# jonasBoss/ndarray-interp

Measured on NVIDIA B200. Metric: queries/s, higher is better.
Workload: dtype f64

## Files before the change

ndarray_interp_b200/csrc/ndi_device.cuh:

```cuda
#pragma once

#include <cuda_runtime.h>
#include <stdint.h>

#include <type_traits>

#include "ndi_internal.h"

namespace ndi {

template <class T> struct Ar;
template <> struct Ar<float> {
    static __device__ __forceinline__ float add(float a, float b) { return __fadd_rn(a, b); }
    static __device__ __forceinline__ float sub(float a, float b) { return __fsub_rn(a, b); }
    static __device__ __forceinline__ float mul(float a, float b) { return __fmul_rn(a, b); }
    static __device__ __forceinline__ float div(float a, float b) { return __fdiv_rn(a, b); }
    static __device__ __forceinline__ float fma(float a, float b, float c) { return __fmaf_rn(a, b, c); }
    static __device__ __forceinline__ bool is_nan(float a) { return a != a; }
    static __device__ __forceinline__ bool is_finite(float a) { return isfinite(a); }
};
template <> struct Ar<double> {
    static __device__ __forceinline__ double add(double a, double b) { return __dadd_rn(a, b); }
    static __device__ __forceinline__ double sub(double a, double b) { return __dsub_rn(a, b); }
    static __device__ __forceinline__ double mul(double a, double b) { return __dmul_rn(a, b); }
// ... 142 lines not shown
struct Slope {
    T d;
    static __device__ __forceinline__ Slope make(T d, T , bool ) { return Slope{d}; }
    __device__ __forceinline__ Slope from_lane(int src) const { return Slope{__shfl_sync(0xffffffffu, d, src)}; }
    __device__ __forceinline__ Slope from_lane(int src, T, bool) const { return from_lane(src); }
};
template <>
struct Slope<float> {
    float d, r;
    static __device__ __forceinline__ Slope make(float d, float dq, bool tables_ok) {
        const bool ok = tables_ok && d >= 0x1p-40f && d <= 0x1p40f && fabsf(dq) <= 0x1p20f * d;
        return Slope{d, ok ? rcp_refined(d) : 0.0f};
    }
    __device__ __forceinline__ Slope from_lane(int src) const {
        return Slope{__shfl_sync(0xffffffffu, d, src), __shfl_sync(0xffffffffu, r, src)};
    }
    __device__ __forceinline__ Slope from_lane(int src, float dq_s, bool tables_ok) const {
#if NDI_PACK_SHFL >= 2
        return make(__shfl_sync(0xffffffffu, d, src), dq_s, tables_ok);
#else
        return from_lane(src);
#endif
    }
};

template <>
struct Slope<double> {
    double d, r;
    static __device__ __forceinline__ Slope make(double d, double , bool enabled) {
        const bool ok = enabled && d >= 0x1p-500 && d <= 0x1p500;
        return Slope{d, ok ? rcp_refined(d) : 0.0};
    }
    __device__ __forceinline__ Slope from_lane(int src) const {
        return Slope{__shfl_sync(0xffffffffu, d, src), __shfl_sync(0xffffffffu, r, src)};
    }
    __device__ __forceinline__ Slope from_lane(int src, double dq_s, bool enabled) const {
#if NDI_PACK_SHFL >= 2
        return make(__shfl_sync(0xffffffffu, d, src), dq_s, enabled);
#else
        return from_lane(src);
#endif
    }
    __device__ __forceinline__ double div(double a) const {
        const double q = div_by(a, d, r);
        return div_ok(a, q) ? q : __ddiv_rn(a, d);
    }
};

template <class T, int V> struct alignas(sizeof(T) * V) Vec { T v[V]; };

template <class T, int V>
__device__ __forceinline__ Vec<T, V> ld_table(const T* p) {
    Vec<T, V> r;
    if constexpr (sizeof(T) * V == 16) {
        int4 t = __ldg(reinterpret_cast<const int4*>(p));
        r = *reinterpret_cast<Vec<T, V>*>(&t);
    } else if constexpr (sizeof(T) * V == 8) {
        int2 t = __ldg(reinterpret_cast<const int2*>(p));
        r = *reinterpret_cast<Vec<T, V>*>(&t);
    } else {
        static_assert(sizeof(T) * V == 4, "unsupported vector width");
        int t = __ldg(reinterpret_cast<const int*>(p));
        r = *reinterpret_cast<Vec<T, V>*>(&t);
    }
    return r;
}
#ifndef NDI_STORE_MODE
#define NDI_STORE_MODE 0
#endif
template <class T, int V>
__device__ __forceinline__ void st_stream(T* p, const Vec<T, V>& r) {
#if NDI_STORE_MODE == 1
    if constexpr (sizeof(T) * V == 16) { *reinterpret_cast<int4*>(p) = *reinterpret_cast<const int4*>(&r); return; }
#elif NDI_STORE_MODE == 2
    if constexpr (sizeof(T) * V == 16) { __stwt(reinterpret_cast<int4*>(p), *reinterpret_cast<const int4*>(&r)); return; }
#elif NDI_STORE_MODE == 3
    if constexpr (sizeof(T) * V == 16) { __stcg(reinterpret_cast<int4*>(p), *reinterpret_cast<const int4*>(&r)); return; }
#endif
    if constexpr (sizeof(T) * V == 16) __stcs(reinterpret_cast<int4*>(p), *reinterpret_cast<const int4*>(&r));
    else if constexpr (sizeof(T) * V == 8) __stcs(reinterpret_cast<int2*>(p), *reinterpret_cast<const int2*>(&r));
    else __stcs(reinterpret_cast<int*>(p), *reinterpret_cast<const int*>(&r));
}
template <class T>
__device__ __forceinline__ T ld_query(const T* p) { return __ldcs(p); }

template <class T, int V>
__device__ __forceinline__ Vec<T, V> lerp_vec(const Vec<T, V>& y1, const Vec<T, V>& y2, const Slope<T>& s, T dq) {
    Vec<T, V> res;
    if constexpr (std::is_same<T, float>::value) {
        if (s.r != 0.0f) {
            if constexpr (NDI_F32X2 && V % 2 == 0) {
                const F2 r2 = F2::both(s.r), nb2 = F2::both(-s.d), dq2 = F2::both(dq);
#pragma unroll
                for (int e = 0; e < V; e += 2) {
                    const F2 a{y1.v[e], y1.v[e + 1]}, b{y2.v[e], y2.v[e + 1]};
                    const F2 o = add_halves(mul2(div_by2(sub2(b, a), nb2, r2), dq2), a);
                    res.v[e] = o.lo; res.v[e + 1] = o.hi;
                }
                return res;
            }
#pragma unroll
            for (int e = 0; e < V; ++e) {
                const float m = div_by(__fsub_rn(y2.v[e], y1.v[e]), s.d, s.r);
                res.v[e] = __fadd_rn(__fmul_rn(m, dq), y1.v[e]);
            }
            return res;
        }
    }
    if constexpr (std::is_same<T, double>::value) {
        if (s.r != 0.0) {
#pragma unroll
            for (int e = 0; e < V; ++e) res.v[e] = __dadd_rn(__dmul_rn(s.div(__dsub_rn(y2.v[e], y1.v[e])), dq), y1.v[e]);
            return res;
        }
    }
#pragma unroll
    for (int e = 0; e < V; ++e) res.v[e] = calc_frac_pre<T>(y1.v[e], y2.v[e], s.d, dq);
    return res;
}

template <class T, int V, bool PACK = true>
__device__ __forceinline__ Vec<T, V> bilerp_vec(const Vec<T, V>& z11, const Vec<T, V>& z12, const Vec<T, V>& z21,
                                                const Vec<T, V>& z22, const Slope<T>& sx, T dqx, const Slope<T>& sy, T dqy) {
    Vec<T, V> res;
    if constexpr (std::is_same<T, float>::value) {
        if (sx.r != 0.0f && sy.r != 0.0f) {
            bool all_ok = true;
            if constexpr (NDI_F32X2 && PACK && V % 2 == 0) {
                const F2 rx = F2::both(sx.r), nbx = F2::both(-sx.d), ry = F2::both(sy.r), nby = F2::both(-sy.d);
                const F2 dx2 = F2::both(dqx), dy2 = F2::both(dqy);
#pragma unroll
                for (int e = 0; e < V; e += 2) {
// ... 298 lines not shown
```

ndarray_interp_b200/csrc/ndi_eval.cu:

```cuda
#include <initializer_list>

#include "ndi_device.cuh"
#include "ndi_internal.h"

namespace ndi {

constexpr int kBlock = 256;
constexpr int kWarpsPerBlock = kBlock / 32;

template <class T>
struct Eval1 {
    const T* grid; int n; SearchCfg sc;
    const T* data; const T* a; const T* b; long long w;
    const T* q; long long nq; int mode;
    T* out; unsigned long long* err;
    long long ntasks; int nslices;
    int fast_tables;
};
template <class T>
struct Eval2 {
    const T* gx; int n; SearchCfg scx;
    const T* gy; int m; SearchCfg scy;
    const T* data; long long w;
    const T* qx; const T* qy; long long nq; int extrapolate;
// ... 252 lines not shown
    const long long want = (total + 255) / 256, cap = (long long)device_info().sm_count * 16;
    pack_pairs_kernel<T><<<(unsigned)(want < cap ? (want ? want : 1) : cap), 256, 0, st>>>(y, (long long)n, (long long)w, P);
    count_launch();
    return cudaGetLastError();
}
bool pair_table_shape_ok(int64_t w, size_t elem) {
    const int64_t v = 16 / (int64_t)elem;
    const int64_t lanes = w / v;
    return w % v == 0 && (lanes == 1 || lanes == 2 || lanes == 4);
}

template <class T>
__device__ __forceinline__ T rem_euclid(T a, T b) {
    T r = fmod(a, b);
    return r < (T)0 ? Ar<T>::add(r, fabs(b)) : r;
}

template <class T>
__device__ __forceinline__ T cubic_point(T yl, T yr, T al, T bl, T t, T omt, T tt) {
    const T lin = Ar<T>::add(Ar<T>::mul(omt, yl), Ar<T>::mul(t, yr));
    const T cur = Ar<T>::add(Ar<T>::mul(al, omt), Ar<T>::mul(bl, t));
    return Ar<T>::add(lin, Ar<T>::mul(tt, cur));
}

template <class T, int V>
__device__ __forceinline__ Vec<T, V> cubic_vec(const Vec<T, V>& yl, const Vec<T, V>& yr, const Vec<T, V>& al, const Vec<T, V>& bl,
                                               T t, T omt, T tt) {
    Vec<T, V> res;
    if constexpr (std::is_same<T, float>::value && NDI_F32X2 && V % 2 == 0) {
        const F2 t2 = F2::both(t), o2 = F2::both(omt), tt2 = F2::both(tt);
#pragma unroll
        for (int e = 0; e < V; e += 2) {
            const F2 l{yl.v[e], yl.v[e + 1]}, r{yr.v[e], yr.v[e + 1]}, a{al.v[e], al.v[e + 1]}, b{bl.v[e], bl.v[e + 1]};
            const F2 lin = add_halves(mul2(o2, l), mul2(t2, r));
            const F2 cur = add_halves(mul2(a, o2), mul2(b, t2));
            const F2 o = add_halves(lin, mul2(tt2, cur));
            res.v[e] = o.lo; res.v[e + 1] = o.hi;
        }
        return res;
    }
#pragma unroll
    for (int e = 0; e < V; ++e) res.v[e] = cubic_point<T>(yl.v[e], yr.v[e], al.v[e], bl.v[e], t, omt, tt);
    return res;
}

template <class T>
__device__ __forceinline__ bool cubic_prepare(T& x, T g0, T gl, int mode) {
    const bool inr = in_range(g0, gl, x);
    if (mode == 0) return !inr;
    if (mode == 2 && !inr) x = Ar<T>::add(rem_euclid<T>(Ar<T>::sub(x, g0), Ar<T>::sub(gl, g0)), g0);
    return Ar<T>::is_nan(x);
}

template <class T, int V, int LPQ>
__global__ void __launch_bounds__(kBlock, (sizeof(T) == 4 && LPQ < 32) ? NDI_THIN_MINBLOCKS : 0) interp1d_cubic_kernel(const Eval1<T> p) {
    extern __shared__ __align__(16) unsigned char smem_raw[];
    __shared__ uint64_t bar;
    const GridView<T> g = make_grid_view<T>(p.grid, p.n, p.sc, smem_raw, &bar);
    const T g0 = g.g0, gl = g.gl;
    const T one = (T)1;
    const int lane = threadIdx.x & 31;
    const long long nwarps = (long long)gridDim.x * kWarpsPerBlock;
    const long long task0 = (long long)blockIdx.x * kWarpsPerBlock + (threadIdx.x >> 5);
    T x_ahead = g0;
    if (LPQ < 32 && kTilesCubic == 1 && task0 < p.ntasks && task0 * 32 + lane < p.nq) x_ahead = ld_query(p.q + task0 * 32 + lane);
    for (long long task = task0; task < p.ntasks; task += nwarps) {
        if constexpr (LPQ < 32) {
            constexpr int TPW = kTilesCubic, QPR = 32 / LPQ;
            const long long qbase0 = task * (32 * TPW);
            T x[TPW]; int idx[TPW]; T tq[TPW], omt[TPW], tt[TPW]; bool skip[TPW], bad[TPW];
            if constexpr (TPW == 1) {
                x[0] = x_ahead;
                const long long qn = (task + nwarps) * 32 + lane;
                x_ahead = (task + nwarps < p.ntasks && qn < p.nq) ? ld_query(p.q + qn) : g0;
                bad[0] = cubic_prepare<T>(x[0], g0, gl, p.mode) && qbase0 + lane < p.nq;
            } else {
#pragma unroll
                for (int t = 0; t < TPW; ++t) {
                    const long long qi = qbase0 + t * 32 + lane;
                    const bool live = qi < p.nq;
                    x[t] = live ? ld_query(p.q + qi) : g0;
                    bad[t] = cubic_prepare<T>(x[t], g0, gl, p.mode) && live;
                }
            }
            search_multi<T, TPW>(g, x, idx, tq, omt);
#pragma unroll
            for (int t = 0; t < TPW; ++t) {
                const long long qi = qbase0 + t * 32 + lane;
                const T xl = tq[t], xr = omt[t];
                tq[t] = Ar<T>::div(Ar<T>::sub(x[t], xl), Ar<T>::sub(xr, xl));
                omt[t] = Ar<T>::sub(one, tq[t]);
                tt[t] = Ar<T>::mul(tq[t], omt[t]);
                if (qbase0 + t * 32 < p.nq) report_first_bad(p.err, bad[t], (unsigned long long)qi);
                skip[t] = bad[t] || !(qi < p.nq);
            }
            const int sub = lane % LPQ, qsel = lane / LPQ;
            const long long col = (long long)sub * V;
            const bool colok = col < p.w;
#pragma unroll
            for (int t = 0; t < TPW; ++t) {
                const long long qbase = qbase0 + t * 32;
                if (qbase >= p.nq) break;
                const int idx0 = __shfl_sync(0xffffffffu, idx[t], __ffs(__ballot_sync(0xffffffffu, !skip[t]) | 0x80000000u) - 1);
                const bool one_interval = LPQ > 1 && __all_sync(0xffffffffu, skip[t] || idx[t] == idx0);
                Vec<T, V> yl, yr, al, bl;
                if (one_interval && colok) {
                    const long long ro = (long long)idx0 * p.w + col;
                    yl = ld_table<T, V>(p.data + ro);
                    yr = ld_table<T, V>(p.data + ro + p.w);
                    al = ld_table<T, V>(p.a + ro);
                    bl = ld_table<T, V>(p.b + ro);
                }
#pragma unroll
                for (int r = 0; r < LPQ; ++r) {
                    const int src = r * QPR + qsel;
#if NDI_PACK_SHFL >= 1
                    const int is = __shfl_sync(0xffffffffu, skip[t] ? -1 : idx[t], src);
                    const bool live_s = is >= 0;
#else
                    const int is = __shfl_sync(0xffffffffu, idx[t], src);
                    const bool live_s = !shfl_b(skip[t], src);
#endif
#if NDI_PACK_CUBIC >= 2
                    const T ts = shfl_t(tq[t], src);
                    const T os = Ar<T>::sub(one, ts), tts = Ar<T>::mul(ts, os);
#else
                    const T ts = shfl_t(tq[t], src), os = shfl_t(omt[t], src), tts = shfl_t(tt[t], src);
#endif
                    if (live_s && colok) {
                        if (!one_interval) {
                            const long long ro = (long long)is * p.w + col;
                            yl = ld_table<T, V>(p.data + ro);
                            yr = ld_table<T, V>(p.data + ro + p.w);
                            al = ld_table<T, V>(p.a + ro);
                            bl = ld_table<T, V>(p.b + ro);
                        }
                        st_stream<T, V>(p.out + (qbase + src) * p.w + col, cubic_vec<T, V>(yl, yr, al, bl, ts, os, tts));
                    }
                }
            }
        } else {
            const long long tile = task / p.nslices;
            const int slice = (int)(task - tile * p.nslices);
            const long long qbase = tile * 32;
            const long long qi = qbase + lane;
            const bool live = qi < p.nq;
            T x[1] = {live ? ld_query(p.q + qi) : g0};
            const bool bad = cubic_prepare<T>(x[0], g0, gl, p.mode) && live;
            int idx[1]; T xls[1], xrs[1];
            search_multi<T, 1>(g, x, idx, xls, xrs);
            const T xl = xls[0], xr = xrs[0];
            const T t = Ar<T>::div(Ar<T>::sub(x[0], xl), Ar<T>::sub(xr, xl));
            const T omt = Ar<T>::sub(one, t);
            const T tt = Ar<T>::mul(t, omt);
            if (slice == 0) report_first_bad(p.err, bad, (unsigned long long)qi);
            const bool skip = bad || !live;
            const long long col = ((long long)slice * 32 + lane) * V;
            const bool colok = col < p.w;
            int cur = -1;
            Vec<T, V> yl, yr, al, bl;
            const int nlive = (int)min((long long)32, p.nq - qbase);
            for (int s = 0; s < nlive; ++s) {
                const int is = __shfl_sync(0xffffffffu, idx[0], s);
                const T ts = shfl_t(t, s), os = shfl_t(omt, s), tts = shfl_t(tt, s);
                const bool sk = shfl_b(skip, s);
                if (sk || !colok) continue;
                if (is != cur) {
                    const long long ro = (long long)is * p.w + col;
                    yl = ld_table<T, V>(p.data + ro);
                    yr = ld_table<T, V>(p.data + ro + p.w);
                    al = ld_table<T, V>(p.a + ro);
                    bl = ld_table<T, V>(p.b + ro);
                    cur = is;
                }
                st_stream<T, V>(p.out + (qbase + s) * p.w + col, cubic_vec<T, V>(yl, yr, al, bl, ts, os, tts));
            }
        }
    }
}

__device__ __forceinline__ F2 sub_halves(F2 p, F2 z) { return F2{__fsub_rn(p.lo, z.lo), __fsub_rn(p.hi, z.hi)}; }

template <class T, int ORDER>
__device__ __forceinline__ T cubic_deriv_point(T num, T h, T r) {
    if constexpr (ORDER == 1) return Hoisted<T>::div(num, h, r);
    else return Hoisted<T>::div(Hoisted<T>::div(num, h, r), h, r);
}

template <class T, int V, int ORDER>
__device__ __forceinline__ Vec<T, V> cubic_deriv_vec(const Vec<T, V>& yl, const Vec<T, V>& yr, const Vec<T, V>& al,
                                                     const Vec<T, V>& bl, T t, T omt, T h, T r) {
    const T dmt = Ar<T>::sub(omt, t), tt = Ar<T>::mul(t, omt);
    const T two = (T)2;
    Vec<T, V> res;
    if constexpr (std::is_same<T, float>::value && NDI_F32X2 && V % 2 == 0) {
        const F2 t2 = F2::both(t), o2 = F2::both(omt), d2 = F2::both(dmt), tt2 = F2::both(tt), two2 = F2::both(two);
#pragma unroll
        for (int e = 0; e < V; e += 2) {
            const F2 l{yl.v[e], yl.v[e + 1]}, rr{yr.v[e], yr.v[e + 1]}, a{al.v[e], al.v[e + 1]}, b{bl.v[e], bl.v[e + 1]};
            const F2 cur = add_halves(mul2(a, o2), mul2(b, t2));
            const F2 ba = sub2(b, a);
            F2 num;
            if constexpr (ORDER == 1) num = add_halves(mul2(tt2, ba), add_halves(mul2(d2, cur), sub2(rr, l)));
            else num = mul2(two2, sub_halves(mul2(d2, ba), cur));
            res.v[e] = cubic_deriv_point<T, ORDER>(num.lo, h, r);
            res.v[e + 1] = cubic_deriv_point<T, ORDER>(num.hi, h, r);
        }
        return res;
    }
#pragma unroll
    for (int e = 0; e < V; ++e) {
        const T cur = Ar<T>::add(Ar<T>::mul(al.v[e], omt), Ar<T>::mul(bl.v[e], t));
        const T ba = Ar<T>::sub(bl.v[e], al.v[e]);
        T num;
        if constexpr (ORDER == 1)
            num = Ar<T>::add(Ar<T>::add(Ar<T>::sub(yr.v[e], yl.v[e]), Ar<T>::mul(dmt, cur)), Ar<T>::mul(tt, ba));
        else num = Ar<T>::mul(two, Ar<T>::sub(Ar<T>::mul(dmt, ba), cur));
        res.v[e] = cubic_deriv_point<T, ORDER>(num, h, r);
    }
    return res;
}

template <class T, int V, int LPQ, int ORDER>
__global__ void __launch_bounds__(kBlock) interp1d_cubic_deriv_kernel(const Eval1<T> p) {
    extern __shared__ __align__(16) unsigned char smem_raw[];
    __shared__ uint64_t bar;
    const GridView<T> g = make_grid_view<T>(p.grid, p.n, p.sc, smem_raw, &bar);
    const T g0 = g.g0, gl = g.gl;
    const T one = (T)1;
// ... 407 lines not shown
            const T y = ld_query(qy + i);
            bady = (check == CHECK_IN_RANGE) ? !in_range(gy0, gyl, y) : Ar<T>::is_nan(y);
        }
        if (badx || bady) {
            unsigned long long word = qy ? 2ull * (unsigned long long)i + (badx ? 0ull : 1ull) : (unsigned long long)i;
            first = min(first, word);
        }
    }
#pragma unroll
    for (int o = 16; o > 0; o >>= 1) first = min(first, __shfl_xor_sync(0xffffffffu, first, o));
    if ((threadIdx.x & 31) == 0 && first != ~0ull) atomicMin(err, first);
}

static int pow2ceil(long long v) { int p = 1; while (p < v && p < 32) p <<= 1; return p; }

static bool aligned(const void* p, size_t a) { return ((uintptr_t)p % a) == 0; }

template <class T>
static int pick_vec(long long w, std::initializer_list<const void*> ptrs) {
    constexpr int vmax = 16 / (int)sizeof(T);
    for (int v = vmax; v > 1; v >>= 1) {
        bool ok = (w % v) == 0;
        for (const void* p : ptrs) ok = ok && aligned(p, sizeof(T) * v);
        if (ok) return v;
    }
    return 1;
}

struct Shape { int v; int lpq; int nslices; long long ntasks; };

static Shape pick_shape(long long w, long long nq, int v, int tiles_per_warp) {
    Shape s;
    s.v = v;
    long long groups = (w + v - 1) / v;
    s.lpq = pow2ceil(groups);
    long long tiles = (nq + 31) / 32;
    if (s.lpq == 32) {
        s.nslices = (int)((groups + 31) / 32);
        s.ntasks = tiles * s.nslices;
    } else {
        s.nslices = 1;
        s.ntasks = (tiles + tiles_per_warp - 1) / tiles_per_warp;
    }
    return s;
}

template <class K>
static cudaError_t prep_smem(K kernel, size_t bytes) {
    if (bytes > 30 * 1024) return cudaFuncSetAttribute(kernel, cudaFuncAttributeMaxDynamicSharedMemorySize, (int)bytes);
    return cudaSuccess;
}

template <class K>
static int persistent_grid(K kernel, size_t smem, long long ntasks) {
    int per_sm = 0;
    if (cudaOccupancyMaxActiveBlocksPerMultiprocessor(&per_sm, kernel, kBlock, smem) != cudaSuccess || per_sm < 1) per_sm = 1;
    long long want = (ntasks + kWarpsPerBlock - 1) / kWarpsPerBlock;
    long long cap = (long long)device_info().sm_count * per_sm;
    return (int)(want < cap ? (want < 1 ? 1 : want) : cap);
}

template <class P, class K>
static cudaError_t launch_eval(K kernel, const P& p, size_t smem, cudaStream_t st) {
    cudaError_t e = prep_smem(kernel, smem);
    if (e != cudaSuccess) return e;
    int grid = persistent_grid(kernel, smem, p.ntasks);
    kernel<<<grid, kBlock, smem, st>>>(p);
    count_launch();
    return cudaGetLastError();
}

#define NDI_LPQ_SWITCH(KERNEL, T, V, LPQ, P, SMEM, ST)                                   \
    switch (LPQ) {                                                                        \
    case 1:  return launch_eval(KERNEL<T, V, 1>, P, SMEM, ST);                            \
    case 2:  return launch_eval(KERNEL<T, V, 2>, P, SMEM, ST);                            \
    case 4:  return launch_eval(KERNEL<T, V, 4>, P, SMEM, ST);                            \
    case 8:  return launch_eval(KERNEL<T, V, 8>, P, SMEM, ST);                            \
    case 16: return launch_eval(KERNEL<T, V, 16>, P, SMEM, ST);                           \
    default: return launch_eval(KERNEL<T, V, 32>, P, SMEM, ST);                           \
    }

#define NDI_VEC_SWITCH(KERNEL, T, SH, P, SMEM, ST)                                        \
    if constexpr (sizeof(T) == 4) {                                                       \
        if (SH.v == 4) { NDI_LPQ_SWITCH(KERNEL, T, 4, SH.lpq, P, SMEM, ST) }              \
        if (SH.v == 2) { NDI_LPQ_SWITCH(KERNEL, T, 2, SH.lpq, P, SMEM, ST) }              \
        NDI_LPQ_SWITCH(KERNEL, T, 1, SH.lpq, P, SMEM, ST)                                 \
    } else {                                                                              \
        if (SH.v == 2) { NDI_LPQ_SWITCH(KERNEL, T, 2, SH.lpq, P, SMEM, ST) }              \
        NDI_LPQ_SWITCH(KERNEL, T, 1, SH.lpq, P, SMEM, ST)                                 \
    }

template <class T, int V, int LPQ> constexpr auto bilinear_direct = interp2d_bilinear_kernel<T, V, LPQ, false>;
template <class T, int V, int LPQ> constexpr auto bilinear_binned = interp2d_bilinear_kernel<T, V, LPQ, true>;

template <class T>
cudaError_t launch_interp1d_linear(const T* grid, int64_t n, SearchCfg sc, const T* data, int64_t w, const T* q,
                                   int64_t nq, int extrapolate, T* out, unsigned long long* err, int fast_tables,
                                   const T* pair, cudaStream_t st) {
    if (nq <= 0) return cudaSuccess;
    if (pair && pair_table_shape_ok(w, sizeof(T)) && aligned(out, 16)) {
        const long long tiles = (nq + 31) / 32;
        Eval1<T> p{grid, (int)n, sc, pair, nullptr, nullptr, (long long)w, q, (long long)nq, extrapolate, out, err, tiles, 1, fast_tables};
        const size_t smem = stage_bytes(sc, sizeof(T));
        switch ((int)(w / (16 / (int64_t)sizeof(T)))) {
        case 1: return launch_eval(interp1d_linear_pair_kernel<T, 1>, p, smem, st);
        case 2: return launch_eval(interp1d_linear_pair_kernel<T, 2>, p, smem, st);
        default: return launch_eval(interp1d_linear_pair_kernel<T, 4>, p, smem, st);
        }
    }
    Shape sh = pick_shape(w, nq, pick_vec<T>(w, {data, out}), kTilesLinear);
    Eval1<T> p{grid, (int)n, sc, data, nullptr, nullptr, (long long)w, q, (long long)nq, extrapolate, out, err, sh.ntasks, sh.nslices, fast_tables};
    size_t smem = stage_bytes(sc, sizeof(T));
    NDI_VEC_SWITCH(interp1d_linear_kernel, T, sh, p, smem, st)
}

template <class T>
cudaError_t launch_interp1d_cubic(const T* grid, int64_t n, SearchCfg sc, const T* data, const T* a, const T* b,
                                  int64_t w, const T* q, int64_t nq, int extrap_mode, T* out,
                                  unsigned long long* err, cudaStream_t st) {
    if (nq <= 0) return cudaSuccess;
    Shape sh = pick_shape(w, nq, pick_vec<T>(w, {data, a, b, out}), kTilesCubic);
    Eval1<T> p{grid, (int)n, sc, data, a, b, (long long)w, q, (long long)nq, extrap_mode, out, err, sh.ntasks, sh.nslices, 0};
    size_t smem = stage_bytes(sc, sizeof(T));
    NDI_VEC_SWITCH(interp1d_cubic_kernel, T, sh, p, smem, st)
}

template <class T, int V, int LPQ> constexpr auto cubic_deriv1 = interp1d_cubic_deriv_kernel<T, V, LPQ, 1>;
template <class T, int V, int LPQ> constexpr auto cubic_deriv2 = interp1d_cubic_deriv_kernel<T, V, LPQ, 2>;

template <class T>
cudaError_t launch_interp1d_cubic_deriv(const T* grid, int64_t n, SearchCfg sc, const T* data, const T* a, const T* b,
                                        int64_t w, const T* q, int64_t nq, int extrap_mode, int order, T* out,
                                        unsigned long long* err, cudaStream_t st) {
    if (nq <= 0) return cudaSuccess;
    Shape sh = pick_shape(w, nq, pick_vec<T>(w, {data, a, b, out}), 1);
    Eval1<T> p{grid, (int)n, sc, data, a, b, (long long)w, q, (long long)nq, extrap_mode, out, err, sh.ntasks, sh.nslices, 0};
    size_t smem = stage_bytes(sc, sizeof(T));
    if (order == 1) { NDI_VEC_SWITCH(cubic_deriv1, T, sh, p, smem, st) }
    NDI_VEC_SWITCH(cubic_deriv2, T, sh, p, smem, st)
}

template <class T>
cudaError_t launch_interp1d_linear_slope(const T* grid, int64_t n, SearchCfg sc, const T* data, int64_t w, const T* q,
                                         int64_t nq, int extrapolate, T* out, unsigned long long* err, cudaStream_t st) {
    if (nq <= 0) return cudaSuccess;
    Shape sh = pick_shape(w, nq, pick_vec<T>(w, {data, out}), 1);
    Eval1<T> p{grid, (int)n, sc, data, nullptr, nullptr, (long long)w, q, (long long)nq, extrapolate, out, err, sh.ntasks, sh.nslices, 0};
    size_t smem = stage_bytes(sc, sizeof(T));
    NDI_VEC_SWITCH(interp1d_linear_slope_kernel, T, sh, p, smem, st)
}

template <class T>
cudaError_t launch_interp2d_bilinear(const T* gx, int64_t n, SearchCfg scx, const T* gy, int64_t m, SearchCfg scy,
                                     const T* data, int64_t w, const T* qx, const T* qy, int64_t nq, int extrapolate,
                                     T* out, unsigned long long* err, const unsigned* perm, int fast_tables,
                                     unsigned long long* next_task, cudaStream_t st) {
    if (nq <= 0) return cudaSuccess;
    Shape sh = pick_shape(w, nq, pick_vec<T>(w, {data, out}), kTilesBilinear);
    Eval2<T> p{gx, (int)n, scx, gy, (int)m, scy, data, (long long)w, qx, qy, (long long)nq, extrapolate, out, err, sh.ntasks, sh.nslices, perm, fast_tables, perm ? next_task : nullptr};
    size_t smem = stage_bytes(scx, sizeof(T)) + stage_bytes(scy, sizeof(T));
    if (perm) { NDI_VEC_SWITCH(bilinear_binned, T, sh, p, smem, st) }
    NDI_VEC_SWITCH(bilinear_direct, T, sh, p, smem, st)
}

template <class T>
cudaError_t launch_lower_index(const T* grid, int64_t n, SearchCfg sc, const T* q, int64_t nq, int64_t* idx,
                               unsigned long long* err, cudaStream_t st) {
    if (nq <= 0) return cudaSuccess;
    size_t smem = stage_bytes(sc, sizeof(T));
    cudaError_t e = prep_smem(lower_index_kernel<T>, smem);
    if (e != cudaSuccess) return e;
    long long blocks = (nq + (long long)kBlock * 4 - 1) / ((long long)kBlock * 4);
    long long cap = (long long)device_info().sm_count * 8;
    lower_index_kernel<T><<<(int)(blocks < cap ? blocks : cap), kBlock, smem, st>>>(grid, (int)n, sc, q, (long long)nq,
                                                                                   (long long*)idx, err);
    count_launch();
    return cudaGetLastError();
// ... 49 lines not shown
```

Before: 707.8 million.

## Restructure wide-row cubic path into block-tiled two-phase kernel with 256-bit accesses

For wide rows (one query spread over a full warp), the cubic kernel now runs in two phases. First each thread of the block prepares one query (search, t, omt, tt) into shared memory. Then warps split the 256 queries and column slices between them, reusing loaded table rows when consecutive queries share an interval. It also adds 32-byte vector load/store paths (ld.global.nc.v4.u64 / st.global.cs.v4.u64) and changes the launch grid to one tile per block. The aim is to remove per-query shuffles and redundant searches across slices, at the cost of block-wide syncs and shared-memory traffic.

Result: slower. 688.5 million, median of 6 (-2.7%).

```diff
diff --git a/ndarray_interp_b200/csrc/ndi_device.cuh b/ndarray_interp_b200/csrc/ndi_device.cuh
--- a/ndarray_interp_b200/csrc/ndi_device.cuh
+++ b/ndarray_interp_b200/csrc/ndi_device.cuh
@@ -218,7 +218,11 @@
 template <class T, int V>
 __device__ __forceinline__ Vec<T, V> ld_table(const T* p) {
     Vec<T, V> r;
-    if constexpr (sizeof(T) * V == 16) {
+    if constexpr (sizeof(T) * V == 32) {
+        unsigned long long t[4];
+        asm("ld.global.nc.v4.u64 {%0,%1,%2,%3}, [%4];" : "=l"(t[0]), "=l"(t[1]), "=l"(t[2]), "=l"(t[3]) : "l"(p));
+        r = *reinterpret_cast<Vec<T, V>*>(t);
+    } else if constexpr (sizeof(T) * V == 16) {
         int4 t = __ldg(reinterpret_cast<const int4*>(p));
         r = *reinterpret_cast<Vec<T, V>*>(&t);
     } else if constexpr (sizeof(T) * V == 8) {
@@ -243,7 +247,10 @@
 #elif NDI_STORE_MODE == 3
     if constexpr (sizeof(T) * V == 16) { __stcg(reinterpret_cast<int4*>(p), *reinterpret_cast<const int4*>(&r)); return; }
 #endif
-    if constexpr (sizeof(T) * V == 16) __stcs(reinterpret_cast<int4*>(p), *reinterpret_cast<const int4*>(&r));
+    if constexpr (sizeof(T) * V == 32) {
+        const unsigned long long* u = reinterpret_cast<const unsigned long long*>(&r);
+        asm volatile("st.global.cs.v4.u64 [%0], {%1,%2,%3,%4};" ::"l"(p), "l"(u[0]), "l"(u[1]), "l"(u[2]), "l"(u[3]));
+    } else if constexpr (sizeof(T) * V == 16) __stcs(reinterpret_cast<int4*>(p), *reinterpret_cast<const int4*>(&r));
     else if constexpr (sizeof(T) * V == 8) __stcs(reinterpret_cast<int2*>(p), *reinterpret_cast<const int2*>(&r));
     else __stcs(reinterpret_cast<int*>(p), *reinterpret_cast<const int*>(&r));
 }
diff --git a/ndarray_interp_b200/csrc/ndi_eval.cu b/ndarray_interp_b200/csrc/ndi_eval.cu
--- a/ndarray_interp_b200/csrc/ndi_eval.cu
+++ b/ndarray_interp_b200/csrc/ndi_eval.cu
@@ -328,20 +328,79 @@
     return Ar<T>::is_nan(x);
 }
 
+constexpr int kCubicQB = kBlock;
+template <class T> struct alignas(16) CubicRec { T t, omt, tt; int is; };
+
+template <class T, int V>
+__device__ __forceinline__ void cubic_wide_rows(const Eval1<T>& p, const GridView<T>& g) {
+    static_assert(kCubicQB == kBlock, "phase 1 prepares one query per thread");
+    __shared__ CubicRec<T> recs[kCubicQB];
+    const T g0 = g.g0, gl = g.gl;
+    const T one = (T)1;
+    const int lane = threadIdx.x & 31, warp = threadIdx.x >> 5;
+    const int nsplit = max(1, kWarpsPerBlock / p.nslices);
+    const int units = p.nslices * nsplit;
+    for (long long tile = blockIdx.x; tile < p.ntasks; tile += gridDim.x) {
+        const long long qbase = tile * kCubicQB;
+        {
+            const long long qi = qbase + threadIdx.x;
+            const bool live = qi < p.nq;
+            T x[1] = {live ? ld_query(p.q + qi) : g0};
+            const bool bad = cubic_prepare<T>(x[0], g0, gl, p.mode) && live;
+            int idx[1]; T xls[1], xrs[1];
+            search_multi<T, 1>(g, x, idx, xls, xrs);
+            const T xl = xls[0], xr = xrs[0];
+            const T t = Ar<T>::div(Ar<T>::sub(x[0], xl), Ar<T>::sub(xr, xl));
+            const T omt = Ar<T>::sub(one, t);
+            const T tt = Ar<T>::mul(t, omt);
+            report_first_bad(p.err, bad, (unsigned long long)qi);
+            recs[threadIdx.x] = CubicRec<T>{t, omt, tt, (bad || !live) ? -1 : idx[0]};
+        }
+        __syncthreads();
+        const int nt = (int)min((long long)kCubicQB, p.nq - qbase);
+        for (int u = warp; u < units; u += kWarpsPerBlock) {
+            const int slice = u % p.nslices, part = u / p.nslices;
+            const long long col = ((long long)slice * 32 + lane) * V;
+            if (col >= p.w) continue;
+            const int s1 = (part + 1) * nt / nsplit;
+            int s = part * nt / nsplit;
+            T* o = p.out + (qbase + s) * p.w + col;
+            int cur = -1;
+            Vec<T, V> yl, yr, al, bl;
+            for (; s < s1; ++s, o += p.w) {
+                const CubicRec<T> r = recs[s];
+                if (r.is < 0) continue;
+                if (r.is != cur) {
+                    const long long ro = (long long)r.is * p.w + col;
+                    yl = ld_table<T, V>(p.data + ro);
+                    yr = ld_table<T, V>(p.data + ro + p.w);
+                    al = ld_table<T, V>(p.a + ro);
+                    bl = ld_table<T, V>(p.b + ro);
+                    cur = r.is;
+                }
+                st_stream<T, V>(o, cubic_vec<T, V>(yl, yr, al, bl, r.t, r.omt, r.tt));
+            }
+        }
+        __syncthreads();
+    }
+}
+
 template <class T, int V, int LPQ>
 __global__ void __launch_bounds__(kBlock, (sizeof(T) == 4 && LPQ < 32) ? NDI_THIN_MINBLOCKS : 0) interp1d_cubic_kernel(const Eval1<T> p) {
     extern __shared__ __align__(16) unsigned char smem_raw[];
     __shared__ uint64_t bar;
     const GridView<T> g = make_grid_view<T>(p.grid, p.n, p.sc, smem_raw, &bar);
-    const T g0 = g.g0, gl = g.gl;
-    const T one = (T)1;
-    const int lane = threadIdx.x & 31;
-    const long long nwarps = (long long)gridDim.x * kWarpsPerBlock;
-    const long long task0 = (long long)blockIdx.x * kWarpsPerBlock + (threadIdx.x >> 5);
-    T x_ahead = g0;
-    if (LPQ < 32 && kTilesCubic == 1 && task0 < p.ntasks && task0 * 32 + lane < p.nq) x_ahead = ld_query(p.q + task0 * 32 + lane);
-    for (long long task = task0; task < p.ntasks; task += nwarps) {
-        if constexpr (LPQ < 32) {
+    if constexpr (LPQ == 32) {
+        cubic_wide_rows<T, V>(p, g);
+    } else {
+        const T g0 = g.g0, gl = g.gl;
+        const T one = (T)1;
+        const int lane = threadIdx.x & 31;
+        const long long nwarps = (long long)gridDim.x * kWarpsPerBlock;
+        const long long task0 = (long long)blockIdx.x * kWarpsPerBlock + (threadIdx.x >> 5);
+        T x_ahead = g0;
+        if (kTilesCubic == 1 && task0 < p.ntasks && task0 * 32 + lane < p.nq) x_ahead = ld_query(p.q + task0 * 32 + lane);
+        for (long long task = task0; task < p.ntasks; task += nwarps) {
             constexpr int TPW = kTilesCubic, QPR = 32 / LPQ;
             const long long qbase0 = task * (32 * TPW);
             T x[TPW]; int idx[TPW]; T tq[TPW], omt[TPW], tt[TPW]; bool skip[TPW], bad[TPW];
@@ -414,42 +473,6 @@
                         st_stream<T, V>(p.out + (qbase + src) * p.w + col, cubic_vec<T, V>(yl, yr, al, bl, ts, os, tts));
                     }
                 }
-            }
-        } else {
-            const long long tile = task / p.nslices;
-            const int slice = (int)(task - tile * p.nslices);
-            const long long qbase = tile * 32;
-            const long long qi = qbase + lane;
-            const bool live = qi < p.nq;
-            T x[1] = {live ? ld_query(p.q + qi) : g0};
-            const bool bad = cubic_prepare<T>(x[0], g0, gl, p.mode) && live;
-            int idx[1]; T xls[1], xrs[1];
-            search_multi<T, 1>(g, x, idx, xls, xrs);
-            const T xl = xls[0], xr = xrs[0];
-            const T t = Ar<T>::div(Ar<T>::sub(x[0], xl), Ar<T>::sub(xr, xl));
-            const T omt = Ar<T>::sub(one, t);
-            const T tt = Ar<T>::mul(t, omt);
-            if (slice == 0) report_first_bad(p.err, bad, (unsigned long long)qi);
-            const bool skip = bad || !live;
-            const long long col = ((long long)slice * 32 + lane) * V;
-            const bool colok = col < p.w;
-            int cur = -1;
-            Vec<T, V> yl, yr, al, bl;
-            const int nlive = (int)min((long long)32, p.nq - qbase);
-            for (int s = 0; s < nlive; ++s) {
-                const int is = __shfl_sync(0xffffffffu, idx[0], s);
-                const T ts = shfl_t(t, s), os = shfl_t(omt, s), tts = shfl_t(tt, s);
-                const bool sk = shfl_b(skip, s);
-                if (sk || !colok) continue;
-                if (is != cur) {
-                    const long long ro = (long long)is * p.w + col;
-                    yl = ld_table<T, V>(p.data + ro);
-                    yr = ld_table<T, V>(p.data + ro + p.w);
-                    al = ld_table<T, V>(p.a + ro);
-                    bl = ld_table<T, V>(p.b + ro);
-                    cur = is;
-                }
-                st_stream<T, V>(p.out + (qbase + s) * p.w + col, cubic_vec<T, V>(yl, yr, al, bl, ts, os, tts));
             }
         }
     }
@@ -964,19 +987,19 @@
 }
 
 template <class K>
-static int persistent_grid(K kernel, size_t smem, long long ntasks) {
+static int persistent_grid(K kernel, size_t smem, long long ntasks, int tasks_per_block) {
     int per_sm = 0;
     if (cudaOccupancyMaxActiveBlocksPerMultiprocessor(&per_sm, kernel, kBlock, smem) != cudaSuccess || per_sm < 1) per_sm = 1;
-    long long want = (ntasks + kWarpsPerBlock - 1) / kWarpsPerBlock;
+    long long want = (ntasks + tasks_per_block - 1) / tasks_per_block;
     long long cap = (long long)device_info().sm_count * per_sm;
     return (int)(want < cap ? (want < 1 ? 1 : want) : cap);
 }
 
 template <class P, class K>
-static cudaError_t launch_eval(K kernel, const P& p, size_t smem, cudaStream_t st) {
+static cudaError_t launch_eval(K kernel, const P& p, size_t smem, cudaStream_t st, int tasks_per_block = kWarpsPerBlock) {
     cudaError_t e = prep_smem(kernel, smem);
     if (e != cudaSuccess) return e;
-    int grid = persistent_grid(kernel, smem, p.ntasks);
+    int grid = persistent_grid(kernel, smem, p.ntasks, tasks_per_block);
     kernel<<<grid, kBlock, smem, st>>>(p);
     count_launch();
     return cudaGetLastError();
@@ -1032,8 +1055,22 @@
                                   unsigned long long* err, cudaStream_t st) {
     if (nq <= 0) return cudaSuccess;
     Shape sh = pick_shape(w, nq, pick_vec<T>(w, {data, a, b, out}), kTilesCubic);
+    size_t smem = stage_bytes(sc, sizeof(T));
+    if (sh.lpq == 32) {
+        constexpr int v32 = 32 / (int)sizeof(T);
+        const bool wide32 = w % v32 == 0 && aligned(data, 32) && aligned(a, 32) && aligned(b, 32) && aligned(out, 32);
+        const int v = wide32 ? v32 : sh.v;
+        const long long slices = ((w + v - 1) / v + 31) / 32;
+        Eval1<T> p{grid, (int)n, sc, data, a, b, (long long)w, q, (long long)nq, extrap_mode, out, err,
+                   (nq + kCubicQB - 1) / kCubicQB, (int)slices, 0};
+        if (wide32) return launch_eval(interp1d_cubic_kernel<T, v32, 32>, p, smem, st, 1);
+        if constexpr (sizeof(T) == 4) {
+            if (v == 4) return launch_eval(interp1d_cubic_kernel<T, 4, 32>, p, smem, st, 1);
+        }
+        if (v == 2) return launch_eval(interp1d_cubic_kernel<T, 2, 32>, p, smem, st, 1);
+        return launch_eval(interp1d_cubic_kernel<T, 1, 32>, p, smem, st, 1);
+    }
     Eval1<T> p{grid, (int)n, sc, data, a, b, (long long)w, q, (long long)nq, extrap_mode, out, err, sh.ntasks, sh.nslices, 0};
-    size_t smem = stage_bytes(sc, sizeof(T));
     NDI_VEC_SWITCH(interp1d_cubic_kernel, T, sh, p, smem, st)
 }
 
```

## Split wide-row cubic into dedicated kernel with 256-bit loads/stores and smem records

Applied to the files above, without the earlier changes.

Moves the wide-row (LPQ==32) cubic path into its own kernel. That kernel stages per-query t/omt/tt/index records in shared memory instead of doing several warp shuffles per output row, processes two rows per iteration, and uses 32-byte vector global loads and streaming stores when alignment allows. The goal is fewer shuffles and fewer memory instructions per row of output. It relies on v4.f64/v8.f32 PTX (Blackwell-era) and adds shared-memory traffic plus a fixed minBlocks launch bound.

New measurement: 746.3 million before, 678.6 million after, median of 6. 9.1% lower.

```diff
diff --git a/ndarray_interp_b200/csrc/ndi_device.cuh b/ndarray_interp_b200/csrc/ndi_device.cuh
--- a/ndarray_interp_b200/csrc/ndi_device.cuh
+++ b/ndarray_interp_b200/csrc/ndi_device.cuh
@@ -218,7 +218,14 @@
 template <class T, int V>
 __device__ __forceinline__ Vec<T, V> ld_table(const T* p) {
     Vec<T, V> r;
-    if constexpr (sizeof(T) * V == 16) {
+    if constexpr (sizeof(T) * V == 32 && sizeof(T) == 8) {
+        asm("ld.global.nc.v4.f64 {%0, %1, %2, %3}, [%4];"
+            : "=d"(r.v[0]), "=d"(r.v[1]), "=d"(r.v[2]), "=d"(r.v[3]) : "l"(p));
+    } else if constexpr (sizeof(T) * V == 32) {
+        asm("ld.global.nc.v8.f32 {%0, %1, %2, %3, %4, %5, %6, %7}, [%8];"
+            : "=f"(r.v[0]), "=f"(r.v[1]), "=f"(r.v[2]), "=f"(r.v[3]), "=f"(r.v[4]), "=f"(r.v[5]), "=f"(r.v[6]), "=f"(r.v[7])
+            : "l"(p));
+    } else if constexpr (sizeof(T) * V == 16) {
         int4 t = __ldg(reinterpret_cast<const int4*>(p));
         r = *reinterpret_cast<Vec<T, V>*>(&t);
     } else if constexpr (sizeof(T) * V == 8) {
@@ -243,7 +250,14 @@
 #elif NDI_STORE_MODE == 3
     if constexpr (sizeof(T) * V == 16) { __stcg(reinterpret_cast<int4*>(p), *reinterpret_cast<const int4*>(&r)); return; }
 #endif
-    if constexpr (sizeof(T) * V == 16) __stcs(reinterpret_cast<int4*>(p), *reinterpret_cast<const int4*>(&r));
+    if constexpr (sizeof(T) * V == 32 && sizeof(T) == 8)
+        asm volatile("st.global.cs.v4.f64 [%0], {%1, %2, %3, %4};"
+                     :: "l"(p), "d"(r.v[0]), "d"(r.v[1]), "d"(r.v[2]), "d"(r.v[3]) : "memory");
+    else if constexpr (sizeof(T) * V == 32)
+        asm volatile("st.global.cs.v8.f32 [%0], {%1, %2, %3, %4, %5, %6, %7, %8};"
+                     :: "l"(p), "f"(r.v[0]), "f"(r.v[1]), "f"(r.v[2]), "f"(r.v[3]), "f"(r.v[4]), "f"(r.v[5]), "f"(r.v[6]),
+                        "f"(r.v[7]) : "memory");
+    else if constexpr (sizeof(T) * V == 16) __stcs(reinterpret_cast<int4*>(p), *reinterpret_cast<const int4*>(&r));
     else if constexpr (sizeof(T) * V == 8) __stcs(reinterpret_cast<int2*>(p), *reinterpret_cast<const int2*>(&r));
     else __stcs(reinterpret_cast<int*>(p), *reinterpret_cast<const int*>(&r));
 }
diff --git a/ndarray_interp_b200/csrc/ndi_eval.cu b/ndarray_interp_b200/csrc/ndi_eval.cu
--- a/ndarray_interp_b200/csrc/ndi_eval.cu
+++ b/ndarray_interp_b200/csrc/ndi_eval.cu
@@ -329,7 +329,8 @@
 }
 
 template <class T, int V, int LPQ>
-__global__ void __launch_bounds__(kBlock, (sizeof(T) == 4 && LPQ < 32) ? NDI_THIN_MINBLOCKS : 0) interp1d_cubic_kernel(const Eval1<T> p) {
+__global__ void __launch_bounds__(kBlock, sizeof(T) == 4 ? NDI_THIN_MINBLOCKS : 0) interp1d_cubic_kernel(const Eval1<T> p) {
+    static_assert(LPQ < 32, "wide rows: interp1d_cubic_wide_kernel");
     extern __shared__ __align__(16) unsigned char smem_raw[];
     __shared__ uint64_t bar;
     const GridView<T> g = make_grid_view<T>(p.grid, p.n, p.sc, smem_raw, &bar);
@@ -339,118 +340,150 @@
     const long long nwarps = (long long)gridDim.x * kWarpsPerBlock;
     const long long task0 = (long long)blockIdx.x * kWarpsPerBlock + (threadIdx.x >> 5);
     T x_ahead = g0;
-    if (LPQ < 32 && kTilesCubic == 1 && task0 < p.ntasks && task0 * 32 + lane < p.nq) x_ahead = ld_query(p.q + task0 * 32 + lane);
+    if (kTilesCubic == 1 && task0 < p.ntasks && task0 * 32 + lane < p.nq) x_ahead = ld_query(p.q + task0 * 32 + lane);
     for (long long task = task0; task < p.ntasks; task += nwarps) {
-        if constexpr (LPQ < 32) {
-            constexpr int TPW = kTilesCubic, QPR = 32 / LPQ;
-            const long long qbase0 = task * (32 * TPW);
-            T x[TPW]; int idx[TPW]; T tq[TPW], omt[TPW], tt[TPW]; bool skip[TPW], bad[TPW];
-            if constexpr (TPW == 1) {
-                x[0] = x_ahead;
-                const long long qn = (task + nwarps) * 32 + lane;
-                x_ahead = (task + nwarps < p.ntasks && qn < p.nq) ? ld_query(p.q + qn) : g0;
-                bad[0] = cubic_prepare<T>(x[0], g0, gl, p.mode) && qbase0 + lane < p.nq;
-            } else {
-#pragma unroll
-                for (int t = 0; t < TPW; ++t) {
-                    const long long qi = qbase0 + t * 32 + lane;
-                    const bool live = qi < p.nq;
-                    x[t] = live ? ld_query(p.q + qi) : g0;
-                    bad[t] = cubic_prepare<T>(x[t], g0, gl, p.mode) && live;
-                }
-            }
-            search_multi<T, TPW>(g, x, idx, tq, omt);
+        constexpr int TPW = kTilesCubic, QPR = 32 / LPQ;
+        const long long qbase0 = task * (32 * TPW);
+        T x[TPW]; int idx[TPW]; T tq[TPW], omt[TPW], tt[TPW]; bool skip[TPW], bad[TPW];
+        if constexpr (TPW == 1) {
+            x[0] = x_ahead;
+            const long long qn = (task + nwarps) * 32 + lane;
+            x_ahead = (task + nwarps < p.ntasks && qn < p.nq) ? ld_query(p.q + qn) : g0;
+            bad[0] = cubic_prepare<T>(x[0], g0, gl, p.mode) && qbase0 + lane < p.nq;
+        } else {
 #pragma unroll
             for (int t = 0; t < TPW; ++t) {
                 const long long qi = qbase0 + t * 32 + lane;
-                const T xl = tq[t], xr = omt[t];
-                tq[t] = Ar<T>::div(Ar<T>::sub(x[t], xl), Ar<T>::sub(xr, xl));
-                omt[t] = Ar<T>::sub(one, tq[t]);
-                tt[t] = Ar<T>::mul(tq[t], omt[t]);
-                if (qbase0 + t * 32 < p.nq) report_first_bad(p.err, bad[t], (unsigned long long)qi);
-                skip[t] = bad[t] || !(qi < p.nq);
-            }
-            const int sub = lane % LPQ, qsel = lane / LPQ;
-            const long long col = (long long)sub * V;
-            const bool colok = col < p.w;
-#pragma unroll
-            for (int t = 0; t < TPW; ++t) {
-                const long long qbase = qbase0 + t * 32;
-                if (qbase >= p.nq) break;
-                const int idx0 = __shfl_sync(0xffffffffu, idx[t], __ffs(__ballot_sync(0xffffffffu, !skip[t]) | 0x80000000u) - 1);
-                const bool one_interval = LPQ > 1 && __all_sync(0xffffffffu, skip[t] || idx[t] == idx0);
-                Vec<T, V> yl, yr, al, bl;
-                if (one_interval && colok) {
-                    const long long ro = (long long)idx0 * p.w + col;
-                    yl = ld_table<T, V>(p.data + ro);
-                    yr = ld_table<T, V>(p.data + ro + p.w);
-                    al = ld_table<T, V>(p.a + ro);
-                    bl = ld_table<T, V>(p.b + ro);
-                }
-#pragma unroll
-                for (int r = 0; r < LPQ; ++r) {
-                    const int src = r * QPR + qsel;
+                const bool live = qi < p.nq;
+                x[t] = live ? ld_query(p.q + qi) : g0;
+                bad[t] = cubic_prepare<T>(x[t], g0, gl, p.mode) && live;
+            }
+        }
+        search_multi<T, TPW>(g, x, idx, tq, omt);
+#pragma unroll
+        for (int t = 0; t < TPW; ++t) {
+            const long long qi = qbase0 + t * 32 + lane;
+            const T xl = tq[t], xr = omt[t];
+            tq[t] = Ar<T>::div(Ar<T>::sub(x[t], xl), Ar<T>::sub(xr, xl));
+            omt[t] = Ar<T>::sub(one, tq[t]);
+            tt[t] = Ar<T>::mul(tq[t], omt[t]);
+            if (qbase0 + t * 32 < p.nq) report_first_bad(p.err, bad[t], (unsigned long long)qi);
+            skip[t] = bad[t] || !(qi < p.nq);
+        }
+        const int sub = lane % LPQ, qsel = lane / LPQ;
+        const long long col = (long long)sub * V;
+        const bool colok = col < p.w;
+#pragma unroll
+        for (int t = 0; t < TPW; ++t) {
+            const long long qbase = qbase0 + t * 32;
+            if (qbase >= p.nq) break;
+            const int idx0 = __shfl_sync(0xffffffffu, idx[t], __ffs(__ballot_sync(0xffffffffu, !skip[t]) | 0x80000000u) - 1);
+            const bool one_interval = LPQ > 1 && __all_sync(0xffffffffu, skip[t] || idx[t] == idx0);
+            Vec<T, V> yl, yr, al, bl;
+            if (one_interval && colok) {
+                const long long ro = (long long)idx0 * p.w + col;
+                yl = ld_table<T, V>(p.data + ro);
+                yr = ld_table<T, V>(p.data + ro + p.w);
+                al = ld_table<T, V>(p.a + ro);
+                bl = ld_table<T, V>(p.b + ro);
+            }
+#pragma unroll
+            for (int r = 0; r < LPQ; ++r) {
+                const int src = r * QPR + qsel;
 #if NDI_PACK_SHFL >= 1
-                    const int is = __shfl_sync(0xffffffffu, skip[t] ? -1 : idx[t], src);
-                    const bool live_s = is >= 0;
+                const int is = __shfl_sync(0xffffffffu, skip[t] ? -1 : idx[t], src);
+                const bool live_s = is >= 0;
 #else
-                    const int is = __shfl_sync(0xffffffffu, idx[t], src);
-                    const bool live_s = !shfl_b(skip[t], src);
+                const int is = __shfl_sync(0xffffffffu, idx[t], src);
+                const bool live_s = !shfl_b(skip[t], src);
 #endif
 #if NDI_PACK_CUBIC >= 2
-                    const T ts = shfl_t(tq[t], src);
-                    const T os = Ar<T>::sub(one, ts), tts = Ar<T>::mul(ts, os);
+                const T ts = shfl_t(tq[t], src);
+                const T os = Ar<T>::sub(one, ts), tts = Ar<T>::mul(ts, os);
 #else
-                    const T ts = shfl_t(tq[t], src), os = shfl_t(omt[t], src), tts = shfl_t(tt[t], src);
+                const T ts = shfl_t(tq[t], src), os = shfl_t(omt[t], src), tts = shfl_t(tt[t], src);
 #endif
-                    if (live_s && colok) {
-                        if (!one_interval) {
-                            const long long ro = (long long)is * p.w + col;
-                            yl = ld_table<T, V>(p.data + ro);
-                            yr = ld_table<T, V>(p.data + ro + p.w);
-                            al = ld_table<T, V>(p.a + ro);
-                            bl = ld_table<T, V>(p.b + ro);
-                        }
-                        st_stream<T, V>(p.out + (qbase + src) * p.w + col, cubic_vec<T, V>(yl, yr, al, bl, ts, os, tts));
+                if (live_s && colok) {
+                    if (!one_interval) {
+                        const long long ro = (long long)is * p.w + col;
+                        yl = ld_table<T, V>(p.data + ro);
+                        yr = ld_table<T, V>(p.data + ro + p.w);
+                        al = ld_table<T, V>(p.a + ro);
+                        bl = ld_table<T, V>(p.b + ro);
                     }
-                }
-            }
-        } else {
-            const long long tile = task / p.nslices;
-            const int slice = (int)(task - tile * p.nslices);
-            const long long qbase = tile * 32;
-            const long long qi = qbase + lane;
-            const bool live = qi < p.nq;
-            T x[1] = {live ? ld_query(p.q + qi) : g0};
-            const bool bad = cubic_prepare<T>(x[0], g0, gl, p.mode) && live;
-            int idx[1]; T xls[1], xrs[1];
-            search_multi<T, 1>(g, x, idx, xls, xrs);
-            const T xl = xls[0], xr = xrs[0];
-            const T t = Ar<T>::div(Ar<T>::sub(x[0], xl), Ar<T>::sub(xr, xl));
-            const T omt = Ar<T>::sub(one, t);
-            const T tt = Ar<T>::mul(t, omt);
-            if (slice == 0) report_first_bad(p.err, bad, (unsigned long long)qi);
-            const bool skip = bad || !live;
-            const long long col = ((long long)slice * 32 + lane) * V;
-            const bool colok = col < p.w;
-            int cur = -1;
+                    st_stream<T, V>(p.out + (qbase + src) * p.w + col, cubic_vec<T, V>(yl, yr, al, bl, ts, os, tts));
+                }
+            }
+        }
+    }
+}
+
+template <class T> struct alignas(16) CubRec { T t, omt, tt; int is; };
+
+template <class T, int V>
+__device__ __forceinline__ void cubic_row(T* o, const CubRec<T>& r, int& cur, Vec<T, V>& yl, Vec<T, V>& yr, Vec<T, V>& al,
+                                          Vec<T, V>& bl, const Eval1<T>& p, long long col) {
+    if (r.is < 0) return;
+    if (r.is != cur) {
+        const long long ro = (long long)r.is * p.w + col;
+        yl = ld_table<T, V>(p.data + ro);
+        yr = ld_table<T, V>(p.data + ro + p.w);
+        al = ld_table<T, V>(p.a + ro);
+        bl = ld_table<T, V>(p.b + ro);
+        cur = r.is;
+    }
+    st_stream<T, V>(o, cubic_vec<T, V>(yl, yr, al, bl, r.t, r.omt, r.tt));
+}
+
+template <class T, int VB>
+__global__ void __launch_bounds__(kBlock, 3) interp1d_cubic_wide_kernel(const Eval1<T> p) {
+    constexpr int V = VB / (int)sizeof(T);
+    extern __shared__ __align__(16) unsigned char smem_raw[];
+    __shared__ uint64_t bar;
+    __shared__ CubRec<T> recs[kWarpsPerBlock][32];
+    const GridView<T> g = make_grid_view<T>(p.grid, p.n, p.sc, smem_raw, &bar);
+    const T g0 = g.g0, gl = g.gl;
+    const T one = (T)1;
+    const int lane = threadIdx.x & 31;
+    CubRec<T>* const rec = recs[threadIdx.x >> 5];
+    const long long nwarps = (long long)gridDim.x * kWarpsPerBlock;
+    const long long task0 = (long long)blockIdx.x * kWarpsPerBlock + (threadIdx.x >> 5);
+    for (long long task = task0; task < p.ntasks; task += nwarps) {
+        const long long tile = task / p.nslices;
+        const int slice = (int)(task - tile * p.nslices);
+        const long long qbase = tile * 32;
+        const long long qi = qbase + lane;
+        const bool live = qi < p.nq;
+        T x[1] = {live ? ld_query(p.q + qi) : g0};
+        const bool bad = cubic_prepare<T>(x[0], g0, gl, p.mode) && live;
+        int idx[1]; T xls[1], xrs[1];
+        search_multi<T, 1>(g, x, idx, xls, xrs);
+        const T t = Ar<T>::div(Ar<T>::sub(x[0], xls[0]), Ar<T>::sub(xrs[0], xls[0]));
+        const T omt = Ar<T>::sub(one, t);
+        if (slice == 0) report_first_bad(p.err, bad, (unsigned long long)qi);
+        __syncwarp();
+        rec[lane] = CubRec<T>{t, omt, Ar<T>::mul(t, omt), bad || !live ? -1 : idx[0]};
+        __syncwarp();
+        const long long col = ((long long)slice * 32 + lane) * V;
+        if (col < p.w) {
+            const int nlive = (int)min((long long)32, p.nq - qbase);
+            T* o = p.out + qbase * p.w + col;
+            int cur = -2;
             Vec<T, V> yl, yr, al, bl;
-            const int nlive = (int)min((long long)32, p.nq - qbase);
-            for (int s = 0; s < nlive; ++s) {
-                const int is = __shfl_sync(0xffffffffu, idx[0], s);
-                const T ts = shfl_t(t, s), os = shfl_t(omt, s), tts = shfl_t(tt, s);
-                const bool sk = shfl_b(skip, s);
-                if (sk || !colok) continue;
-                if (is != cur) {
-                    const long long ro = (long long)is * p.w + col;
-                    yl = ld_table<T, V>(p.data + ro);
-                    yr = ld_table<T, V>(p.data + ro + p.w);
-                    al = ld_table<T, V>(p.a + ro);
-                    bl = ld_table<T, V>(p.b + ro);
-                    cur = is;
-                }
-                st_stream<T, V>(p.out + (qbase + s) * p.w + col, cubic_vec<T, V>(yl, yr, al, bl, ts, os, tts));
-            }
+            int s = 0;
+            for (; s + 2 <= nlive; s += 2, o += 2 * p.w) {
+                if (rec[s].is == cur && rec[s + 1].is == cur) {
+                    const CubRec<T> r0 = rec[s], r1 = rec[s + 1];
+                    const Vec<T, V> v0 = cubic_vec<T, V>(yl, yr, al, bl, r0.t, r0.omt, r0.tt);
+                    const Vec<T, V> v1 = cubic_vec<T, V>(yl, yr, al, bl, r1.t, r1.omt, r1.tt);
+                    st_stream<T, V>(o, v0);
+                    st_stream<T, V>(o + p.w, v1);
+                } else {
+                    cubic_row<T, V>(o, rec[s], cur, yl, yr, al, bl, p, col);
+                    cubic_row<T, V>(o + p.w, rec[s + 1], cur, yl, yr, al, bl, p, col);
+                }
+            }
+            if (s < nlive) cubic_row<T, V>(o, rec[s], cur, yl, yr, al, bl, p, col);
         }
     }
 }
@@ -1026,15 +1059,31 @@
     NDI_VEC_SWITCH(interp1d_linear_kernel, T, sh, p, smem, st)
 }
 
+template <class T, int V, int LPQ> constexpr auto cubic_thin = interp1d_cubic_kernel<T, V, LPQ < 32 ? LPQ : 16>;
+
 template <class T>
 cudaError_t launch_interp1d_cubic(const T* grid, int64_t n, SearchCfg sc, const T* data, const T* a, const T* b,
                                   int64_t w, const T* q, int64_t nq, int extrap_mode, T* out,
                                   unsigned long long* err, cudaStream_t st) {
     if (nq <= 0) return cudaSuccess;
     Shape sh = pick_shape(w, nq, pick_vec<T>(w, {data, a, b, out}), kTilesCubic);
+    const size_t smem = stage_bytes(sc, sizeof(T));
+    if (sh.lpq == 32) {
+        constexpr int v32 = 32 / (int)sizeof(T);
+        const bool b32 = w % v32 == 0 && aligned(data, 32) && aligned(a, 32) && aligned(b, 32) && aligned(out, 32);
+        const int v = b32 ? v32 : sh.v;
+        const int nslices = (int)((w / v + 31) / 32);
+        const long long ntasks = (nq + 31) / 32 * nslices;
+        Eval1<T> p{grid, (int)n, sc, data, a, b, (long long)w, q, (long long)nq, extrap_mode, out, err, ntasks, nslices, 0};
+        switch (v * (int)sizeof(T)) {
+        case 32: return launch_eval(interp1d_cubic_wide_kernel<T, 32>, p, smem, st);
+        case 16: return launch_eval(interp1d_cubic_wide_kernel<T, 16>, p, smem, st);
+        case 8:  return launch_eval(interp1d_cubic_wide_kernel<T, 8>, p, smem, st);
+        default: return launch_eval(interp1d_cubic_wide_kernel<T, sizeof(T)>, p, smem, st);
+        }
+    }
     Eval1<T> p{grid, (int)n, sc, data, a, b, (long long)w, q, (long long)nq, extrap_mode, out, err, sh.ntasks, sh.nslices, 0};
-    size_t smem = stage_bytes(sc, sizeof(T));
-    NDI_VEC_SWITCH(interp1d_cubic_kernel, T, sh, p, smem, st)
+    NDI_VEC_SWITCH(cubic_thin, T, sh, p, smem, st)
 }
 
 template <class T, int V, int LPQ> constexpr auto cubic_deriv1 = interp1d_cubic_deriv_kernel<T, V, LPQ, 1>;
```
